# christophersanborn/Radiative3D

Measured on AMD Instinct MI355X. Metric: phonon-histories/sec, higher is better.
Workload: dtype f64

## Files before the change

### __graft_entry__.py

```python
import os
import subprocess
import sys

REPO = os.path.dirname(os.path.abspath(__file__))
if REPO not in sys.path:
    sys.path.insert(0, REPO)


def build():
    env = dict(os.environ)
    env.setdefault("HIPCC", "/opt/rocm/bin/hipcc")
    subprocess.check_call(["make", "-C", REPO, "-j", str(min(8, os.cpu_count() or 1)), "all"], env=env)
    subprocess.check_call(["make", "-C", REPO, "variant", "NAME=STEPFINALS", "DEFS=-DR3D_STEP_FINALS=1"], env=env,
                          stdout=subprocess.DEVNULL)
    subprocess.check_call(["g++", "-std=c++17", "-O2", "-fPIC", "-shared", "-o",
                           os.path.join(REPO, "tests", "emul", "libr3d_emul.so"),
                           os.path.join(REPO, "tests", "emul", "emul.cpp")])
    import radiative3d_amd
    from radiative3d_amd import _ffi
    _ffi.host_lib()
    for so in ("libr3d_hip.so", "libr3d_host.so"):
        if not os.path.exists(os.path.join(_ffi.LIBDIR, so)):
            raise RuntimeError(f"{so} was not produced")


def smoke():
    import torch
    from radiative3d_amd import Engine, Model
    from radiative3d_amd.parallel import DeviceResult
    from oracle import oracle_ffi
    from radiative3d_amd.configs import crustpinch

    from oracle.check import assert_aggregates_equal_without, forked_ids

    n = 4096
    model = Model(crustpinch(4))
    engine = Engine(model, device=0)
    got, gf = engine.run(n, first_id=0, seed=0x5EED, trace=True)
    want, wf = oracle_ffi.run(model, n, first_id=0, seed=0x5EED, trace=True)
    assert got.n_lost + got.n_timeout + got.n_invalid == n
    forked = forked_ids(gf, wf, 0)
    assert len(forked) <= n // 1000, f"{len(forked)} of {n} histories differ from the oracle: ids {forked}"

    def same_as_oracle(r, what):
        assert_aggregates_equal_without(r, want, forked, lambda k, i: engine.run(k, i, 0x5EED),
                                        lambda k, i: oracle_ffi.run(model, k, i, 0x5EED), what)

    same_as_oracle(got, "diagnostic kernel")
    same_as_oracle(engine.run(n, first_id=0, seed=0x5EED), "production kernel")
    total = DeviceResult(model, "cuda:0")
    engine.run_device(n // 2, 0, 0x5EED, *total.pointers(), carry="carry")
    engine.run_device(n - n // 2, n // 2, 0x5EED, *total.pointers(), carry="carry")
    engine.run_device(0, 0, 0x5EED, *total.pointers(), carry="final")
    torch.cuda.synchronize()
    same_as_oracle(total.to_result(), "carry chain + drain kernel")
    import ctypes as C
    from radiative3d_amd import Node, _ffi
    from radiative3d_amd.parallel import Comm
    node = Node(model, [0])
    same_as_oracle(node.run(n, first_id=0, seed=0x5EED), "r3d_node_run")
    node.close()
    L = _ffi.hip_lib()
    ident = C.create_string_buffer(_ffi.R3D_COMM_ID_BYTES)
    assert L.r3d_comm_unique_id(ident) == 0, L.r3d_last_error().decode()
    handle = L.r3d_comm_create(ident, 0, 1, 0)
    assert handle, L.r3d_last_error().decode()
    comm = Comm(handle, L)
    assert comm.describe()["n_ranks"] == 1
    comm.reduce_(total.energy, total.counts, total.scalars)
    comm.reduce_(total.energy, total.counts, total.scalars, root=0)
    torch.cuda.synchronize()
    same_as_oracle(total.to_result(), "block after r3d_comm_reduce")
    comm.close()
    print(f"smoke ok: {n} histories, {len(forked)} differ from the oracle (diagnostic, self-contained, chain-step and drain kernels), "
          f"kernel {engine.last_kernel_ms():.3f} ms")
    engine.close()


if __name__ == "__main__":
    build()
    if len(sys.argv) > 1 and sys.argv[1] == "smoke":
        smoke()
```

Measured before the change: 1.386 billion.

## Add specialized tetrahedral pool step kernel with neighbor-cell prefetch

Adds a dedicated tetrahedral-cell step body that specializes the pool_kernel template for CELL_TET. It fetches the neighbor cell's face normals and offsets early, using vectorized 16-byte loads, while the current move is still being computed. It also keeps a lane moving across several cell transfers before returning it to the queues. The goal is to hide global-memory latency on cell records and to cut queue round-trips, at the cost of more code and register pressure. The build step also adds a reproducible STEPFINALS variant.

```diff
diff --git a/__graft_entry__.py b/__graft_entry__.py
--- a/__graft_entry__.py
+++ b/__graft_entry__.py
@@ -12,6 +12,9 @@
     env.setdefault("HIPCC", "/opt/rocm/bin/hipcc")
     subprocess.check_call(["make", "-C", REPO, "-j", str(min(8, os.cpu_count() or 1)), "all"], env=env)
     subprocess.check_call(["make", "-C", REPO, "variant", "NAME=STEPFINALS", "DEFS=-DR3D_STEP_FINALS=1"], env=env,
+                          stdout=subprocess.DEVNULL)
+    subprocess.check_call(["make", "-C", REPO, "variant", "NAME=STEPFINALS_REPRO",
+                           "DEFS=-DR3D_STEP_FINALS=1 -DR3D_REPRODUCIBLE -ffp-contract=off"], env=env,
                           stdout=subprocess.DEVNULL)
     subprocess.check_call(["g++", "-std=c++17", "-O2", "-fPIC", "-shared", "-o",
                            os.path.join(REPO, "tests", "emul", "libr3d_emul.so"),
diff --git a/radiative3d_amd/tet_step/r3d_kernels_tet.hip b/radiative3d_amd/tet_step/r3d_kernels_tet.hip
--- /dev/null
+++ b/radiative3d_amd/tet_step/r3d_kernels_tet.hip
@@ -0,0 +1,74 @@
+#include <hip/hip_runtime.h>
+
+#include <type_traits>
+
+#include "../../include/r3d.h"
+#include "../csrc/r3d_kernels.h"
+#include "../csrc/r3d_pool.h"
+#include "r3d_tet_step.h"
+
+namespace r3d {
+
+template <>
+__global__ __launch_bounds__(kPoolBlock) void pool_kernel<CELL_TET, false, true, false>(const KArgs a) {
+  tet_step::step_body<true>(a);
+}
+template <>
+__global__ __launch_bounds__(kPoolBlock) void pool_kernel<CELL_TET, false, false, false>(const KArgs a) {
+  tet_step::step_body<false>(a);
+}
+
+namespace {
+
+constexpr int K = CELL_TET;
+
+template <class F>
+hipError_t with_res(int res, F&& f) {
+  if (res == RES_NONE) return f(std::false_type{});
+  return f(std::true_type{});
+}
+
+}
+
+hipError_t launch_pool_tet(int res, bool trace, bool drain_only, unsigned grid, size_t lds_bytes, hipStream_t s,
+                           const KArgs& a) {
+  return with_res(res, [&](auto scat) {
+    constexpr bool H = decltype(scat)::value;
+    if (drain_only && !trace)
+      hipLaunchKernelGGL((pool_drain_kernel<K, false, H>), dim3(grid), dim3(kPoolBlock), lds_bytes, s, a);
+    else if (trace)
+      hipLaunchKernelGGL((pool_kernel<K, false, H, true>), dim3(grid), dim3(kPoolBlock), lds_bytes, s, a);
+    else if (a.carry_out)
+      hipLaunchKernelGGL((pool_kernel<K, false, H, false>), dim3(grid), dim3(kPoolBlock), lds_bytes, s, a);
+    else
+      hipLaunchKernelGGL((pool_job_kernel<K, false, H>), dim3(grid), dim3(kPoolBlock), lds_bytes, s, a);
+    return hipGetLastError();
+  });
+}
+
+hipError_t pool_lds_attr_tet(int res, int lds_bytes) {
+  return with_res(res, [&](auto scat) {
+    constexpr bool H = decltype(scat)::value;
+    hipError_t r = hipFuncSetAttribute(reinterpret_cast<const void*>(&pool_kernel<K, false, H, false>),
+                                       hipFuncAttributeMaxDynamicSharedMemorySize, lds_bytes);
+    if (r != hipSuccess) return r;
+    r = hipFuncSetAttribute(reinterpret_cast<const void*>(&pool_drain_kernel<K, false, H>),
+                            hipFuncAttributeMaxDynamicSharedMemorySize, lds_bytes);
+    if (r != hipSuccess) return r;
+    r = hipFuncSetAttribute(reinterpret_cast<const void*>(&pool_job_kernel<K, false, H>),
+                            hipFuncAttributeMaxDynamicSharedMemorySize, lds_bytes);
+    if (r != hipSuccess) return r;
+    return hipFuncSetAttribute(reinterpret_cast<const void*>(&pool_kernel<K, false, H, true>),
+                               hipFuncAttributeMaxDynamicSharedMemorySize, lds_bytes);
+  });
+}
+
+#ifdef R3D_PHASE_TIMING
+int pool_stats_tet(unsigned long long out[40]) {
+  if (hipMemcpyFromSymbol(out, HIP_SYMBOL(g_pool_stats), 40 * sizeof(unsigned long long)) != hipSuccess) return 1;
+  unsigned long long zero[40] = {};
+  return hipMemcpyToSymbol(HIP_SYMBOL(g_pool_stats), zero, sizeof zero) != hipSuccess;
+}
+#endif
+
+}
diff --git a/radiative3d_amd/tet_step/r3d_tet_step.h b/radiative3d_amd/tet_step/r3d_tet_step.h
--- /dev/null
+++ b/radiative3d_amd/tet_step/r3d_tet_step.h
@@ -0,0 +1,640 @@
+#ifndef R3D_TET_STEP_H_
+#define R3D_TET_STEP_H_
+
+#include <stddef.h>
+
+#include "../csrc/r3d_pool.h"
+
+namespace r3d {
+namespace tet_step {
+
+typedef double d2v __attribute__((ext_vector_type(2)));
+typedef uint32_t u4v __attribute__((ext_vector_type(4)));
+typedef __attribute__((address_space(1))) const d2v gd2;
+typedef __attribute__((address_space(1))) const u4v gu4;
+static_assert(offsetof(CellTet, g) == 0 && offsetof(CellTet, v0) == 24 && offsetof(CellTet, inv_gmag) == 32 &&
+              offsetof(CellTet, att) == 40 && offsetof(CellTet, n) == 48 && offsetof(CellTet, d) == 144 &&
+              offsetof(CellTet, link) == 176, "the pieces below follow CellTet's layout");
+
+__device__ __forceinline__ void fetch_normals(CellTet& c, const CellTet* rec) {
+  gd2* r = (gd2*)rec;
+  const d2v q3 = r[3], q4 = r[4], q5 = r[5], q6 = r[6], q7 = r[7], q8 = r[8];
+  c.n[0][0] = q3.x, c.n[0][1] = q3.y, c.n[0][2] = q4.x;
+  c.n[1][0] = q4.y, c.n[1][1] = q5.x, c.n[1][2] = q5.y;
+  c.n[2][0] = q6.x, c.n[2][1] = q6.y, c.n[2][2] = q7.x;
+  c.n[3][0] = q7.y, c.n[3][1] = q8.x, c.n[3][2] = q8.y;
+}
+__device__ __forceinline__ void fetch_offsets(CellTet& c, const CellTet* rec) {
+  gd2* r = (gd2*)rec;
+  const d2v q9 = r[9], q10 = r[10];
+  const u4v l = ((gu4*)rec)[11];
+  c.d[0] = q9.x, c.d[1] = q9.y, c.d[2] = q10.x, c.d[3] = q10.y;
+  c.link[0] = l.x, c.link[1] = l.y, c.link[2] = l.z, c.link[3] = l.w;
+}
+#ifndef R3D_TET_EARLY_OFFSETS
+#define R3D_TET_EARLY_OFFSETS 1
+#endif
+__device__ __forceinline__ void fetch_planes(CellTet& c, const CellTet* rec) {
+  fetch_normals(c, rec);
+  fetch_offsets(c, rec);
+}
+__device__ __forceinline__ void fetch_early(CellTet& c, const CellTet* rec) {
+  fetch_normals(c, rec);
+  if (R3D_TET_EARLY_OFFSETS) fetch_offsets(c, rec);
+}
+__device__ __forceinline__ void fetch_late(CellTet& c, const CellTet* rec) {
+  if (!R3D_TET_EARLY_OFFSETS) fetch_offsets(c, rec);
+}
+__device__ __forceinline__ void fetch_head(CellTet& c, const CellTet* rec) {
+  gd2* r = (gd2*)rec;
+  const d2v q0 = r[0], q1 = r[1], q2 = r[2];
+  c.g[0] = q0.x, c.g[1] = q0.y, c.g[2] = q1.x, c.v0 = q1.y;
+  c.inv_gmag = q2.x, c.att = q2.y;
+}
+
+__device__ __forceinline__ uint32_t pick_link(const CellTet& c, int f) {
+  const uint32_t l0 = c.link[0], l1 = c.link[1], l2 = c.link[2], l3 = c.link[3];
+  return f == 0 ? l0 : f == 1 ? l1 : f == 2 ? l2 : l3;
+}
+__device__ __forceinline__ V3 pick_normal(const CellTet& c, int f) {
+  const V3 n0 = v3(c.n[0]), n1 = v3(c.n[1]), n2 = v3(c.n[2]), n3 = v3(c.n[3]);
+  V3 r;
+  r.x = f == 0 ? n0.x : f == 1 ? n1.x : f == 2 ? n2.x : n3.x;
+  r.y = f == 0 ? n0.y : f == 1 ? n1.y : f == 2 ? n2.y : n3.y;
+  r.z = f == 0 ? n0.z : f == 1 ? n1.z : f == 2 ? n2.z : n3.z;
+  return r;
+}
+
+__device__ __forceinline__ int tet_move(const KArgs& a, const Tables<CELL_TET>& T, CellTet& c, Phonon& p, Rng& rng,
+                                        LaneStats& st, int* reason, Pending& ev, bool may_repeat, bool& fetched,
+                                        V3& fnorm) {
+  fetched = false;
+  if (p.t > a.ttl) return FATE_TIMEOUT;
+  if ((p.moves & 127u) == 127u) {
+    if (isnan(p.path)) return *reason = 0, FATE_INVALID;
+    if (isnan(p.t)) return *reason = 1, FATE_INVALID;
+    if (p.path < 0) return *reason = 2, FATE_INVALID;
+    if (p.t < 0 || p.recent < 0) return *reason = 3, FATE_INVALID;
+    if (p.recent == 0) return *reason = 4, FATE_INVALID;
+    if (p.recent < a.slow_concern) return *reason = 5, FATE_INVALID;
+    if (p.moves > a.loop_concern) return *reason = 6, FATE_INVALID;
+    p.recent = 0;
+  }
+  st.iterations++;
+  R3D_SCHED_FENCE();
+  double u_free = rng_draw(rng, rng_key(a.seed));
+  asm volatile("" : "+v"(u_free));
+  R3D_SCHED_FENCE();
+
+  Exit e;
+  bool scatters = false, slow;
+  uint32_t lk;
+  int scat;
+  e.len = 0.0;
+  {
+    TetLocal L;
+    const TetFast F = tet_fast_exit(c, p, L);
+    slow = !F.ok;
+    e.face = F.face;
+    lk = pick_link(c, e.face);
+    scat = cell_scat(c);
+    fnorm = pick_normal(c, e.face);
+    const uint32_t lf = tet_link_flags(lk);
+    fetched = may_repeat && !slow && (lf & F_ADJOIN) && !(lf & (F_COLLECT | F_REFLECT | F_DISCON));
+    if (fetched) {
+      const CellTet* next = T.cells + (2 * tet_link_neighbor(lk) + p.type);
+      asm volatile("" : "+v"(next));
+      fetch_early(c, next);
+    }
+    R3D_SCHED_FENCE();
+    if (!slow) {
+      e.len = L.R * two_atan(F.t, F.sn, F.cs);
+      asm volatile("" : "+v"(e.len), "+v"(scat));
+      const double mfp = T.scat_head[scat].mfp[p.type];
+      double scatlen = pos_inf();
+      if (!((1.0 - u_free) * mfp >= e.len)) scatlen = -log_lean(u_free) * mfp;
+      scatters = scatlen < e.len;
+      double len = e.len, sn = F.sn, cs = F.cs, omc = F.omc;
+      if (any_lanes(scatters)) {
+        if (scatters) {
+          len = scatlen;
+          rotation(len * frcp(L.R), &sn, &cs);
+          omc = (sn * sn) * frcp(1.0 + cs);
+        }
+      }
+      tet_advance_local(c, L, p, len, sn, cs, omc);
+    }
+  }
+  if (any_lanes(slow)) {
+    if (slow) {
+      const TetSlowOut o = tet_move_reference_inline(&cell_rec<CELL_TET>(T, p.cell, p.type), p, u_free,
+                                                     T.scat_head[scat].mfp[p.type]);
+      if (o.fate != FATE_ALIVE) return o.fate;
+      p = o.p, e.face = o.face, scatters = o.scatters != 0;
+      lk = pick_link(c, e.face);
+      fnorm = pick_normal(c, e.face);
+    }
+  }
+  ev.face = scatters ? -1 : e.face;
+  ev.flags = scatters ? 0u : tet_link_flags(lk);
+  ev.nbr = scatters ? -1 : tet_link_neighbor(lk);
+  ev.vel = 0.0;
+  return FATE_ALIVE;
+}
+
+__device__ __forceinline__ bool tet_hand_over(const KArgs& a, const Tables<CELL_TET>& T, CellTet& c, Phonon& p,
+                                              LaneStats& st, const Pending& ev, V3 fnorm, bool may_repeat) {
+  const int nbr = ev.nbr, ty = p.type;
+  const uint32_t fl = ev.flags;
+  const double vi = cell_velocity(c, p.loc, ty);
+  if (may_repeat) fetch_late(c, T.cells + (2 * nbr + ty));
+  if (may_repeat || !(fl & F_SMOOTH)) fetch_head(c, T.cells + (2 * nbr + ty));
+  R3D_SCHED_FENCE();
+  bool crossed = true;
+  if (!(fl & F_SMOOTH)) {
+    const double vo = cell_velocity(c, p.loc, ty);
+    bool step = (fl & F_STEP) != 0;
+    if (!step) {
+      const double ui = velocity_in<CELL_TET>(T, p.cell, p.loc, 1 - ty), uo = velocity_in<CELL_TET>(T, nbr, p.loc, 1 - ty);
+      const double v1 = ty == RAY_P ? vi : ui, v2 = ty == RAY_P ? vo : uo;
+      const double w1 = ty == RAY_P ? ui : vi, w2 = ty == RAY_P ? uo : vo;
+      double dvp = fabs(2 * (v2 - v1) / (v2 + v1));
+      double dvs = fabs(2 * (w2 - w1) / (w2 + w1));
+      step = (dvp > dvs ? dvp : dvs) > 0.00001;
+    }
+    if (step) crossed = bend<false>(p, cell_face_normal(cell_rec<CELL_TET>(T, p.cell, ty), ev.face, p.loc), vi, vo);
+  }
+  if (crossed) {
+    p.cell = nbr, st.transfer++;
+  } else {
+    st.reflect++;
+    volume_count(a, p, st);
+  }
+  return crossed;
+}
+
+template <bool LDS_SCAT>
+__device__ __forceinline__ void step_body(const KArgs& a) {
+  constexpr int KIND = CELL_TET;
+  using Cell = CellTet;
+  extern __shared__ __align__(16) unsigned char smem[];
+  const unsigned tid = threadIdx.x, lane = tid & 63u;
+
+  {
+    auto copy_words = [&](void* dst, const void* src, size_t bytes) {
+      unsigned long long* d = reinterpret_cast<unsigned long long*>(dst);
+      const unsigned long long* s = reinterpret_cast<const unsigned long long*>(src);
+      for (size_t i = tid; i < bytes / 8; i += kPoolBlock) d[i] = s[i];
+    };
+    if (LDS_SCAT) {
+      copy_words(smem + a.lds_scat_off, a.scat_head, (size_t)a.n_scat * sizeof(ScatHead));
+      copy_words(smem + a.lds_scatptr_off, a.scat_ptrs, (size_t)a.n_scat * sizeof(ScatPtrs));
+    }
+    if (a.acc_bits) {
+      const size_t n = (size_t)1 << a.acc_bits;
+      unsigned long long* z = reinterpret_cast<unsigned long long*>(smem + a.lds_acc_off);
+      for (size_t i = tid; i < n * 5; i += kPoolBlock) z[i] = 0ull;
+      uint32_t* k = reinterpret_cast<uint32_t*>(smem + a.lds_acc_off + n * 5 * sizeof(double));
+      for (size_t i = tid; i < n * 3; i += kPoolBlock) k[i] = (i < n) ? kEmpty : 0u;
+    }
+  }
+  BinCache bc;
+  bc.on = a.acc_bits != 0;
+  bc.e = reinterpret_cast<double*>(smem + a.lds_acc_off);
+  bc.key = reinterpret_cast<uint32_t*>(smem + a.lds_acc_off + ((size_t)5 * sizeof(double) << a.acc_bits));
+  bc.cnt = bc.key + ((size_t)1 << a.acc_bits);
+  bc.mask = (1u << a.acc_bits) - 1u, bc.shift = 32u - a.acc_bits;
+  Tables<KIND> T;
+  T.cells = reinterpret_cast<const Cell*>(a.cells);
+  T.scat_head = LDS_SCAT ? reinterpret_cast<const ScatHead*>(smem + a.lds_scat_off) : a.scat_head;
+  T.scat_ptrs = LDS_SCAT ? reinterpret_cast<const ScatPtrs*>(smem + a.lds_scatptr_off) : a.scat_ptrs;
+  T.seis_scan = a.seis_scan;
+  T.seis_hit = a.seis_hit;
+
+  const uint32_t S = a.pool_slots, rcap = a.pool_ring_mask + 1u, rmask = a.pool_ring_mask;
+  const uint32_t rlog = 31u - (uint32_t)__builtin_clz(rcap);
+  constexpr uint32_t F = kSlotStride;
+  struct alignas(16) D2 { double a, b; };
+  struct alignas(16) U4 { uint32_t a, b, c, d; };
+  enum { P_T_PATH, P_RECENT_LAMP, P_LX_LY, P_LZ_DX, P_DY_DZ, P_PC_PS, P_NUM };
+  enum { U_STATE , U_ID , U_NUM };
+  static_assert((P_NUM + U_NUM) * 16 == kSlotBytes, "slot layout");
+  D2* const pd = reinterpret_cast<D2*>(smem + a.lds_pool_off);
+  U4* const pu = reinterpret_cast<U4*>(pd + (size_t)P_NUM * F);
+  lds_u16* const rings = (lds_u16*)(smem + a.lds_ring_off);
+  __shared__ PoolCtl ctl;
+  __shared__ unsigned long long s_tally[R3D_N_SCALARS];
+  for (uint32_t i = tid; i < Q_NUM * rcap; i += kPoolBlock) rings[i] = kRingEmpty;
+  if (tid < R3D_N_SCALARS) s_tally[tid] = 0ull;
+  if (tid < 8) ctl.word[tid] = 0u, ctl.tail[tid] = 0u;
+  __syncthreads();
+  auto ring = [&](int q) { return rings + (uint32_t)q * rcap; };
+  const size_t image_words = (size_t)F * (kSlotBytes / 4);
+  if (a.carry_in) {
+    const uint32_t* img = reinterpret_cast<const uint32_t*>(a.carry_in) + (size_t)blockIdx.x * image_words;
+    uint32_t* dst = reinterpret_cast<uint32_t*>(pd);
+    for (size_t i = tid; i < image_words; i += kPoolBlock) dst[i] = img[i];
+    __syncthreads();
+    for (uint32_t base = 0; base < S; base += kPoolBlock) {
+      const uint32_t s = base + tid;
+      const bool have = s < S;
+      const int tag = have ? (int)((pu[U_STATE * F + s].d >> 16) & 7u) : 0;
+      q_push_all(ctl, rings, rcap, rlog, lane, have, tag, s);
+    }
+  } else {
+    for (uint32_t s = tid; s < S; s += kPoolBlock) {
+      ring(Q_FREE)[s] = (uint16_t)s;
+      pu[U_STATE * F + s].d = meta_pack(0, -1, 0u, Q_FREE);
+    }
+    if (tid == 0) ctl.tail[Q_FREE] = S, ctl.word[Q_FREE] = S;
+  }
+  __syncthreads();
+
+  constexpr int kEv = 3 + R3D_INV_NUM;
+  auto tally_n = [&](int slot, unsigned long long n) {
+    if (lane == 0 && n) atomicAdd(&s_tally[slot], n);
+  };
+  auto tally = [&](bool cond, int slot) { tally_n(slot, (unsigned long long)__popcll(ballot(cond))); };
+  auto count = [&](bool cond) { return (uint32_t)__popcll(ballot(cond)); };
+  auto finish = [&](bool died, int fate, int reason, const Phonon& p, unsigned slot) {
+    if (!any_lane(died)) return;
+    tally(died && fate == FATE_LOST, 0);
+    tally(died && fate == FATE_TIMEOUT, 1);
+    if (any_lane(died && fate == FATE_INVALID)) {
+      tally(died && fate == FATE_INVALID, 2);
+#pragma unroll
+      for (int r = 0; r < R3D_INV_NUM; r++) tally(died && fate == FATE_INVALID && reason == r, 3 + r);
+    }
+    if (R3D_STEP_FINALS) {
+      if (a.pfinals) {
+        if (died) {
+          const U4 ids = pu[U_ID * F + slot];
+          r3d_final* f = reinterpret_cast<r3d_final*>(a.pfinals) + (((uint64_t)ids.b << 32) | ids.a);
+          f->time = p.t, f->path = p.path, f->amp = p.lamp;
+          f->loc[0] = p.loc.x, f->loc[1] = p.loc.y, f->loc[2] = p.loc.z;
+          f->dir[0] = p.dir.x, f->dir[1] = p.dir.y, f->dir[2] = p.dir.z;
+          f->moves = p.moves;
+          f->fate = (uint8_t)fate;
+          f->type = (uint8_t)p.type;
+          f->n_catch = (uint16_t)0xFFFFu;
+        }
+      }
+    }
+  };
+  auto load_state = [&](unsigned id, Phonon& p, Rng& rng, uint32_t& meta, uint32_t& nbr) {
+    const D2* d = pd + id;
+    const D2 q0 = d[P_T_PATH * F], q1 = d[P_RECENT_LAMP * F], q2 = d[P_LX_LY * F], q3 = d[P_LZ_DX * F],
+             q4 = d[P_DY_DZ * F], q5 = d[P_PC_PS * F];
+    const U4 u0 = pu[U_STATE * F + id], u1 = pu[U_ID * F + id];
+    p.t = q0.a, p.path = q0.b, p.recent = q1.a, p.lamp = q1.b;
+    p.loc = v3(q2.a, q2.b, q3.a);
+    p.dir = v3(q3.b, q4.a, q4.b);
+    p.pc = q5.a, p.ps = q5.b;
+    p.cell = (int32_t)u0.a, p.moves = u0.b, rng.k = u0.c, meta = u0.d;
+    p.type = (int32_t)(meta & 1u);
+    rng.id_lo = u1.a, rng.id_hi = u1.b, nbr = u1.d;
+  };
+  auto store_event = [&](unsigned id, const Phonon& p, const Rng& rng, uint32_t meta) {
+    D2* d = pd + id;
+    d[P_LZ_DX * F].b = p.dir.x;
+    d[P_DY_DZ * F] = D2{p.dir.y, p.dir.z}, d[P_PC_PS * F] = D2{p.pc, p.ps};
+    pu[U_STATE * F + id] = U4{(uint32_t)p.cell, p.moves, rng.k, meta};
+  };
+  auto store_state = [&](unsigned id, const Phonon& p, const Rng& rng, uint32_t meta) {
+    D2* d = pd + id;
+    d[P_T_PATH * F] = D2{p.t, p.path}, d[P_RECENT_LAMP * F] = D2{p.recent, p.lamp};
+    d[P_LX_LY * F] = D2{p.loc.x, p.loc.y}, d[P_LZ_DX * F] = D2{p.loc.z, p.dir.x};
+    d[P_DY_DZ * F] = D2{p.dir.y, p.dir.z}, d[P_PC_PS * F] = D2{p.pc, p.ps};
+    pu[U_STATE * F + id] = U4{(uint32_t)p.cell, p.moves, rng.k, meta};
+  };
+#ifdef R3D_PHASE_TIMING
+  __shared__ unsigned long long s_stats[5][8];
+  if (tid < 40) s_stats[tid / 8][tid % 8] = 0ull;
+  __syncthreads();
+#endif
+
+  typedef const __attribute__((address_space(4))) KArgs* KernArgs;
+  KernArgs args = (KernArgs)__builtin_amdgcn_kernarg_segment_ptr();
+  unsigned k_chain = 0;
+  int dest = Q_FREE;
+  unsigned id = 0;
+  for (;;) {
+    asm volatile("" : "+s"(args));
+    const KArgs& a = *(const KArgs*)args;
+    int q;
+    unsigned k;
+    bool act;
+#ifdef R3D_PHASE_TIMING
+    unsigned long long t_pop = __builtin_readcyclecounter();
+#endif
+    if (k_chain) {
+      const unsigned kc = (unsigned)__builtin_amdgcn_readfirstlane((int)k_chain);
+      q = (int)(kc >> 8), k = kc & 0xFFu, act = lane < k;
+      k_chain = 0;
+    } else {
+      const uint32_t snap = lane < 8 ? lds_ld(&ctl.word[lane]) : 0u;
+      const uint32_t drained = (uint32_t)__builtin_amdgcn_readlane((int)snap, kDrainedWord);
+      if (drained && a.carry_out) break;
+      const uint32_t cnt = snap & 0xFFFFu;
+      const bool minor = lane == (unsigned)Q_RT || lane == (unsigned)Q_COLLECT || lane == (unsigned)Q_SCATTER;
+      uint32_t full = (uint32_t)ballot(cnt >= (minor ? kMinorFull : 64u)) & ((1u << Q_NUM) - 1u);
+      if (drained) {
+        if ((uint32_t)__builtin_amdgcn_readlane((int)cnt, Q_FREE) == S) break;
+        full &= ~(1u << Q_FREE);
+      }
+      q = (full & (1u << Q_RT)) ? Q_RT : (full & (1u << Q_COLLECT)) ? Q_COLLECT : (full & (1u << Q_SCATTER)) ? Q_SCATTER
+          : (full & (1u << Q_FREE)) ? Q_FREE : (full & (1u << Q_MOVE)) ? Q_MOVE : -1;
+      if (q < 0) {
+        uint32_t best = 0u;
+#pragma unroll
+        for (int j = 0; j < Q_NUM; j++) {
+          const uint32_t cj = (drained && j == Q_FREE) ? 0u : (uint32_t)__builtin_amdgcn_readlane((int)cnt, j);
+          if (cj > best) best = cj, q = j;
+        }
+      }
+      if (q < 0) {
+#ifdef R3D_PHASE_TIMING
+        if (lane == 0) atomicAdd(&s_stats[0][6], 1ull);
+#endif
+        R3D_PRIO_LOW();
+        __builtin_amdgcn_s_sleep(8);
+        continue;
+      }
+      const uint32_t wq = (uint32_t)__builtin_amdgcn_readlane((int)snap, q);
+      R3D_PRIO_HIGH();
+      k = q_pop(ctl, ring(q), rmask, rlog, q, lane, wq, id);
+      if (k == 0) {
+        R3D_PRIO_LOW();
+        continue;
+      }
+      act = lane < k;
+    }
+    const bool thin = k < 64u;
+#ifdef R3D_PHASE_TIMING
+    const unsigned long long t_begin = __builtin_readcyclecounter();
+#endif
+    dest = Q_FREE;
+    uint32_t n_iter = 0, n_transfer = 0, n_reflect = 0;
+    uint32_t n_volout = 0;
+
+    if (q == Q_FREE) R3D_PRIO_LOW();
+    if (q == Q_FREE) {
+      const unsigned want = k;
+      unsigned long long base = 0;
+      if (lane == 0) base = atomicAdd(a.next, (unsigned long long)want);
+      base = ((unsigned long long)(uint32_t)__builtin_amdgcn_readlane((int)(base >> 32), 0) << 32) |
+             (uint32_t)__builtin_amdgcn_readlane((int)base, 0);
+      const unsigned take = base >= a.n ? 0u : (a.n - base < want ? (unsigned)(a.n - base) : want);
+      if (take < want && lane == 0)
+        __hip_atomic_store(&ctl.word[kDrainedWord], 1u, __ATOMIC_RELAXED, __HIP_MEMORY_SCOPE_WORKGROUP);
+      const bool fresh = lane < take;
+      if (fresh) {
+        Phonon p;
+        Rng rng;
+        rng_init(rng, a.first_id + base + lane);
+        spray(a, p, rng);
+        store_state(id, p, rng, meta_pack(p.type, -1, 0u, Q_MOVE));
+        pu[U_ID * F + id] = U4{rng.id_lo, rng.id_hi, 0u, 0u};
+      }
+      dest = fresh ? Q_MOVE : dest;
+      tally_n(kEv + R3D_EV_GENERATED, take);
+    } else if (q == Q_MOVE) {
+      Phonon p = {};
+      Rng rng = {};
+      Cell c;
+      bool have = false;
+      uint32_t meta = 0;
+      int fate = FATE_ALIVE, reason = 0;
+      bool live = act;
+      U4 u0 = U4{0u, 0u, 0u, 0u};
+      if (act) u0 = pu[U_STATE * F + id];
+      {
+        const Cell* rec = T.cells + (2 * (int32_t)u0.a + (int32_t)(u0.d & 1u));
+        fetch_planes(c, rec);
+        fetch_head(c, rec);
+      }
+      R3D_SCHED_FENCE();
+      if (act) {
+        const D2* d = pd + id;
+        const D2 q0 = d[P_T_PATH * F], q1 = d[P_RECENT_LAMP * F], q2 = d[P_LX_LY * F], q3 = d[P_LZ_DX * F],
+                 q4 = d[P_DY_DZ * F], q5 = d[P_PC_PS * F];
+        const U4 u1 = pu[U_ID * F + id];
+        p.t = q0.a, p.path = q0.b, p.recent = q1.a, p.lamp = q1.b;
+        p.loc = v3(q2.a, q2.b, q3.a);
+        p.dir = v3(q3.b, q4.a, q4.b);
+        p.pc = q5.a, p.ps = q5.b;
+        p.cell = (int32_t)u0.a, p.moves = u0.b, rng.k = u0.c, meta = u0.d;
+        p.type = (int32_t)(meta & 1u);
+        rng.id_lo = u1.a, rng.id_hi = u1.b;
+        have = true;
+        R3D_PRIO_MOVE();
+      }
+      (void)meta;
+#pragma nounroll
+      for (int rep = 0;; rep++) {
+        Pending ev;
+        ev.vel = 0.0, ev.face = -1, ev.flags = 0u, ev.nbr = -1;
+        bool leaving = false, fetched = false;
+        V3 fnorm = v3(0, 0, 0);
+        LaneStats st = {0, 0, 0, 0, 0, 0, 0, 0, 0};
+        asm volatile("" : "+v"(id), "+v"(rng.id_lo), "+v"(rng.id_hi), "+v"(p.type));
+        if (any_lanes(live && !have)) {
+          if (live && !have) {
+            const Cell* rec = T.cells + (2 * p.cell + p.type);
+            fetch_planes(c, rec);
+            fetch_head(c, rec);
+          }
+        }
+        const bool may_repeat = thin ? rep + 1 < kPoolMovesThin : rep + 1 < kPoolMoves;
+        if (live) {
+          fate = tet_move(a, T, c, p, rng, st, &reason, ev, may_repeat, fetched, fnorm);
+          leaving = true;
+          if (fate != FATE_ALIVE) {
+            dest = Q_FREE;
+          } else if (ev.face < 0) {
+            dest = Q_SCATTER;
+          } else if (ev.flags & F_COLLECT) {
+            dest = Q_COLLECT;
+          } else if (!(ev.flags & (F_REFLECT | F_ADJOIN))) {
+            dest = Q_FREE, fate = FATE_LOST;
+          } else if (ev.flags & (F_REFLECT | F_DISCON)) {
+            dest = Q_RT;
+          } else {
+            leaving = false;
+          }
+        }
+        const bool light = live && !leaving;
+        have = false;
+        if (light) {
+          if (!fetched && may_repeat) fetch_early(c, T.cells + (2 * ev.nbr + p.type));
+          have = tet_hand_over(a, T, c, p, st, ev, fnorm, may_repeat) && may_repeat;
+        }
+        n_iter += count(st.iterations != 0u), n_transfer += count(st.transfer != 0u), n_reflect += count(st.reflect != 0u);
+        if (a.vol) n_volout += count(st.vol_out != 0u);
+        live = light;
+        const unsigned n_live = (unsigned)__popcll(ballot(live));
+        const bool last = !thin ? (rep + 1 >= kPoolMoves) || (n_live < kMoveAgainLanes)
+                                : (rep + 1 >= kPoolMovesThin) || (n_live == 0u);
+#ifdef R3D_PHASE_TIMING
+        if (lane == 0) atomicAdd(&s_stats[0][7], 1ull), atomicAdd(&s_stats[1][7], (unsigned long long)(n_live));
+#endif
+        if (last && live) dest = Q_MOVE;
+        if (leaving || (last && live)) {
+          const bool keep = dest != Q_FREE;
+          if (keep) {
+            store_state(id, p, rng, meta_pack(p.type, dest == Q_MOVE ? -1 : ev.face, dest == Q_MOVE ? 0u : ev.flags, dest));
+            if (dest == Q_RT || dest == Q_COLLECT)
+              pu[U_ID * F + id].d = (uint32_t)ev.nbr;
+          } else
+            pu[U_STATE * F + id].d = meta_pack(0, -1, 0u, Q_FREE);
+        }
+        if (last) break;
+      }
+      const bool died = act && dest == Q_FREE;
+      finish(died, fate, reason, p, id);
+    } else if (q == Q_COLLECT) {
+      Phonon p = {};
+      Rng rng = {};
+      uint32_t meta = 0, nbr = 0;
+      uint32_t k0 = 0, k1 = 0, catches = 0;
+      double vel = 1.0;
+      Pending ev;
+      ev.vel = 0.0, ev.face = 0, ev.flags = 0u, ev.nbr = -1;
+      if (act) {
+        load_state(id, p, rng, meta, nbr);
+        R3D_PRIO_LOW();
+        ev.face = (int)((meta >> 1) & 7u) - 1, ev.flags = (meta >> 8) & 0xFFu;
+        vel = velocity_in<KIND>(T, p.cell, p.loc, p.type);
+        const SeisGrid& g = a.grid;
+        const double fx = (p.loc.x - g.origin[0]) * g.inv_h;
+        const double fy = (p.loc.y - g.origin[1]) * g.inv_h;
+        const double fz = (p.loc.z - g.origin[2]) * g.inv_h;
+        if (fx >= 0 && fy >= 0 && fz >= 0 && fx < g.dim_f[0] && fy < g.dim_f[1] && fz < g.dim_f[2]) {
+          const int cellid = ((int)fz * g.dim[1] + (int)fy) * g.dim[0] + (int)fx;
+          k0 = g.start[cellid], k1 = g.start[cellid + 1];
+        }
+      }
+#ifdef R3D_ABLATE_COLLECT
+      k1 = k0;
+#endif
+      tally_n(kEv + R3D_EV_COLLECT, k);
+      if (any_lane(k1 > k0)) {
+        const uint32_t hits = pool_collect_pairs<KIND, false>(a, T, p, vel, k0, k1, nullptr, lane, catches, bc);
+        tally_n(kEv + R3D_EV_CATCH, hits);
+      }
+      bool died = false;
+      if (act) {
+        if (!(ev.flags & (F_REFLECT | F_ADJOIN))) {
+          died = true;
+        } else if (ev.flags & (F_REFLECT | F_DISCON)) {
+          dest = Q_RT;
+        } else {
+          dest = Q_MOVE;
+        }
+      }
+      const bool light = act && dest == Q_MOVE;
+      LaneStats st = {0, 0, 0, 0, 0, 0, 0, 0, 0};
+      if (light) step_event<KIND, EV_BEND>(a, T, p, rng, st, ev, (int)nbr);
+      n_transfer += count(st.transfer != 0u), n_reflect += count(st.reflect != 0u);
+      if (a.vol) n_volout += count(st.vol_out != 0u);
+      if (act) {
+        const uint32_t m2 = died ? meta_pack(0, -1, 0u, Q_FREE)
+                                 : meta_pack(p.type, light ? -1 : ev.face, light ? 0u : ev.flags, dest);
+        if (light) store_event(id, p, rng, m2);
+        else pu[U_STATE * F + id].d = m2;
+      }
+      finish(died, FATE_LOST, 0, p, id);
+    } else {
+      Phonon p = {};
+      Rng rng = {};
+      uint32_t meta = 0, nbr = 0;
+      LaneStats st = {0, 0, 0, 0, 0, 0, 0, 0, 0};
+      if (act) {
+        load_state(id, p, rng, meta, nbr);
+        R3D_PRIO_LOW();
+        Pending ev;
+        ev.vel = 0.0, ev.face = (int)((meta >> 1) & 7u) - 1, ev.flags = (meta >> 8) & 0xFFu, ev.nbr = -1;
+        if (q == Q_RT) {
+#ifdef R3D_ABLATE_RT
+          step_event<KIND, EV_RT>(a, T, p, rng, st, ev, (int)nbr);
+#else
+          const RtChoice ch = rt_event_choose<KIND>(a, T, p, rng, st, ev, (int)nbr);
+          const uint32_t draws = rng.k;
+          asm volatile("" ::: "memory");
+          load_state(id, p, rng, meta, nbr);
+          rng.k = draws;
+          Pending ev2;
+          ev2.vel = 0.0, ev2.face = (int)((meta >> 1) & 7u) - 1, ev2.flags = (meta >> 8) & 0xFFu, ev2.nbr = -1;
+          rt_event_apply<KIND>(a, T, p, st, ev2, (int)nbr, ch);
+#endif
+        } else {
+          step_event<KIND, EV_SCATTER>(a, T, p, rng, st, ev);
+        }
+        store_event(id, p, rng, meta_pack(p.type, -1, 0u, Q_MOVE));
+        dest = Q_MOVE;
+      }
+      if (q == Q_RT) n_transfer += count(st.transfer != 0u), n_reflect += count(st.reflect != 0u);
+      if (a.vol) n_volout += count(st.vol_out != 0u);
+    }
+    if (q == Q_SCATTER) tally_n(kEv + R3D_EV_SCATTER, k);
+    tally_n(kEv + R3D_EV_ITERATIONS, n_iter), tally_n(kEv + R3D_EV_TRANSFER, n_transfer);
+    tally_n(kEv + R3D_EV_REFLECT, n_reflect);
+    tally_n(kEv + R3D_EV_VOLUME_OUT, n_volout);
+    tally_n(kEv + R3D_EV_RTSOLVE, q == Q_RT ? k : 0u);
+#ifdef R3D_PHASE_TIMING
+    const unsigned long long t_push = __builtin_readcyclecounter();
+#endif
+    R3D_PRIO_HIGH();
+    if (q == Q_COLLECT && k == 64u && !any_lane(act && dest != Q_RT)) {
+      k_chain = (unsigned)__builtin_amdgcn_readfirstlane((int)(k | ((unsigned)Q_RT << 8)));
+    } else if (q == Q_RT || q == Q_SCATTER) {
+      k_chain = (unsigned)__builtin_amdgcn_readfirstlane((int)(k | ((unsigned)Q_MOVE << 8)));
+    } else {
+      q_push_all(ctl, rings, rcap, rlog, lane, act, dest, id);
+    }
+#ifdef R3D_PHASE_TIMING
+    if (lane == 0) {
+      const unsigned long long t_end = __builtin_readcyclecounter();
+      atomicAdd(&s_stats[0][q], 1ull);
+      atomicAdd(&s_stats[1][q], (unsigned long long)k);
+      atomicAdd(&s_stats[2][q], t_end - t_pop);
+      atomicAdd(&s_stats[3][q], t_begin - t_pop);
+      atomicAdd(&s_stats[4][q], t_end - t_push);
+    }
+#endif
+  }
+
+  __syncthreads();
+  asm volatile("" : "+s"(args));
+  const KArgs& a_end = *(const KArgs*)args;
+  if (a_end.carry_out) {
+    uint32_t* img = reinterpret_cast<uint32_t*>(a_end.carry_out) + (size_t)blockIdx.x * image_words;
+    const uint32_t* src = reinterpret_cast<const uint32_t*>(pd);
+    for (size_t i = tid; i < image_words; i += kPoolBlock) img[i] = src[i];
+  }
+  if (bc.on) {
+    for (uint32_t i = tid; i <= bc.mask; i += kPoolBlock) {
+      const uint32_t bin = bc.key[i];
+      if (bin == kEmpty) continue;
+      double* e = a_end.energy + (size_t)bin * 5;
+#pragma unroll
+      for (int cc = 0; cc < 5; cc++) {
+        const double v = bc.e[i * 5u + cc];
+        if (v != 0.0) unsafeAtomicAdd(e + cc, v);
+      }
+#pragma unroll
+      for (int t = 0; t < 2; t++) {
+        const uint32_t n = bc.cnt[i * 2u + t];
+        if (n) atomicAdd(a_end.counts + (size_t)bin * 2 + t, (unsigned long long)n);
+      }
+    }
+  }
+#ifdef R3D_PHASE_TIMING
+  if (tid < 40) atomicAdd(&g_pool_stats[tid / 8][tid % 8], s_stats[tid / 8][tid % 8]);
+#endif
+  if (tid < R3D_N_SCALARS && s_tally[tid] != 0ull) atomicAdd(a_end.scalars + tid, s_tally[tid]);
+}
+
+}
+}
+#endif
```

Result: slower. 1.150 billion (-17.0%).
